# K1nght/Unified-Unlearning-w-Remain-Geometry

Hardware: AMD Instinct MI355X
Metric: SFR-on unlearning steps/sec, DiT-XL/2 256px bs32/GPU (higher is better)
Workload: dtype bf16

## Files before the change

include/sfron.h:

```cpp
#ifndef SFRON_H
#define SFRON_H
#include <stdint.h>
#ifdef __cplusplus
extern "C" {
#endif

int sfron_abi_version(void);
const char* sfron_build_arch(void);


int sfron_sweep_partials_len(void);

int sfron_sumsq_masked(const float* g, const float* g2, const uint8_t* mask, int64_t n, double* partials, int* nblk_out,
                       void* stream);

int sfron_sumsq_masked_ranges(const float* g, const uint8_t* mask, const int64_t* ranges, int n_ranges, double* partials, void* stream);

int sfron_clip_coef(const double* partials, int nblk, float max_norm, float* stats, void* stream);

int sfron_masked_clip_adam(float* p, const float* g, const float* g2 , float* m, float* v,
                           const uint8_t* mask, const float* stats,
                           int64_t n, double beta1, double beta2, double eps, double step_size, double bc2_sqrt,
                           double decay_mul, uint16_t* w_bf16, float* ema, double ema_decay, int ema_mode, void* stream);

// ... 39 lines not shown
int sfron_ddpm_alphas_cumprod(const float* betas, int T, float* abar, void* stream);
int sfron_ddpm_q_sample(const float* x0, const float* e, const int64_t* t, const float* abar, int n, int chw, float* x_t,
                        void* stream);
int sfron_ddpm_sample_loss(const float* e, const float* model_out, int n, int chw, float* per_sample, void* stream);
int sfron_ddpm_loss_coef(const float* per_sample, int n, int mode, float lambd, float scale, int n_global, float* wsum,
                         int use_wsum, float* coef, float* loss, void* stream);
int sfron_ddpm_loss_bwd(const float* e, const float* model_out, const float* coef, int n, int chw, float* d_model_out,
                        void* stream);
int sfron_ddim_step(const float* x, const float* eps, const float* noise, int64_t n, float s1, float s2, float s3, float c1,
                    float c2, float* x_next, float* x0_pred, void* stream);
int sfron_ddim_cfg_step(const float* x, const float* eps_uncond, const float* eps_cond, const float* noise, int64_t n, float guidance,
                        float sqrt_one_minus_at, float sqrt_at, float sqrt_a_prev, float dir_coef, float sigma, float* x_prev, float* pred_x0,
                        void* stream);

enum {
  SFRON_EPI_BF16 = 0,
  SFRON_EPI_F32 = 1,
  SFRON_EPI_GELU = 2,
  SFRON_EPI_GATE_RES = 3,
  SFRON_EPI_DGELU = 4,
  SFRON_EPI_POS = 5,
  SFRON_EPI_GELU_Q = 7,
  SFRON_EPI_DGELU_Q = 8,
  SFRON_EPI_QUICK_GELU = 9
};
typedef struct sfron_gemm_desc {
  const uint16_t* A; const uint16_t* B;
  int M, N, K, lda, ldb;
  int a_transposed, b_transposed;
  int epilogue;
  float alpha;
  const float* bias;
  uint16_t* c_bf16; int ldc_bf16;
  float* c_f32; int ldc_f32;
  uint16_t* aux; int ldaux;
  const float* gate; int ldgate;
  const float* pos;
  int tokens;
  int accumulate;
  const float* resid;
  int split_k;
  long split_stride;
  int tile_hint;
  float* a_rowsum;
  float* rowsum_ws;
  float* col_partials;
  const uint8_t* sumsq_mask;
  double* sumsq_partials;
} sfron_gemm_desc;
int sfron_gemm_bf16(const sfron_gemm_desc* desc , void* stream);
int sfron_gemm_dgelu_colpart_rows(int M, int N, int K);
int sfron_gemm_gelu_q_supported(int M, int N, int K);
int sfron_gemm_rowsum_supported(int M, int N, int K);
int sfron_split_sum_bf16(const float* slabs, int n_splits, int64_t n, int64_t split_stride, uint16_t* out, void* stream);
int sfron_split_gate_res(const float* slabs, int n_splits, int64_t split_stride, const float* bias, const float* gate, int ldgate, int tokens,
                         const float* resid, float* out, uint16_t* branch, int M, int N, void* stream);

int sfron_gemm_sumsq_partials(int M, int N, int K);



int sfron_fp8_quant_tensors(const float* params, const int64_t* table, int n_tensors, const float* scales, uint32_t* amax_bits,
                            uint8_t* dst, int mode, void* stream);
int sfron_fp8_update_scales(uint32_t* amax_bits, int n_tensors, float* scales, void* stream);
int sfron_fp8_activation_amax(uint32_t* act_amax, float* out3 , int reset, void* stream);

int sfron_cast_e4m3(const void* src, int src_is_bf16, int64_t n, float scale, uint8_t* dst, uint32_t* act_amax ,
                    void* stream);
int sfron_ln_modulate_fwd_q(const float* x, const float* shift, const float* scale, int ldmod, int tokens, int M, int D, uint16_t* out,
                            uint8_t* out_e4m3, float e4m3_scale, float* mean, float* rstd, uint32_t* act_amax ,
                            void* stream);

typedef struct sfron_fp8_gemm_desc {
  const uint8_t* A; const uint8_t* B;
  int M, N, K;
  const float* w_scale;
  float a_scale;
  int epilogue;
  const float* bias;
  uint16_t* c_bf16; int ldc_bf16;
  uint16_t* aux; int ldaux;
  uint8_t* c_e4m3; float c_e4m3_scale;
  float* c_f32; int ldc_f32;
  const float* resid;
  const float* gate; int ldgate;
  int tokens;
  uint32_t* act_amax;
  int aux_q;
} sfron_fp8_gemm_desc;
int sfron_fp8_gemm_supported(int M, int N, int K);
int sfron_fp8_gemm(const sfron_fp8_gemm_desc* desc , void* stream);

int sfron_cast_mx8(const uint16_t* src, int M, int N, uint8_t* dst, uint8_t* scales, void* stream);
int sfron_fp8_transpose_shadow(const uint8_t* w8, uint8_t* w8t, const int64_t* table, int n_matrices, void* stream);
typedef struct sfron_fp8_dgrad_desc {
  const uint8_t* A;
  const uint8_t* a_scales;
  const uint8_t* B;
  int M, N, K;
  const float* w_scale;
  int epilogue;
  uint16_t* c_bf16; int ldc_bf16;
  const uint16_t* aux; int ldaux;
  uint8_t* c_e4m3;
  uint8_t* c_scales;
  float* col_partials;
// ... 315 lines not shown
```

unified-unlearning-w-remain-geometry_amd/_lib.py:

```python
import ctypes
import os
from ctypes import POINTER, c_char_p, c_double, c_float, c_int, c_int64, c_void_p

_HERE = os.path.dirname(os.path.abspath(__file__))
LIB_PATH = os.path.join(_HERE, "libsfron.so")


class SfronError(RuntimeError):
    pass


_lib = None
ABI_VERSION = 16

_P = c_void_p
_S = c_void_p

_PROTOS = {
    "sfron_abi_version": (c_int, []),
    "sfron_build_arch": (c_char_p, []),
    "sfron_sweep_partials_len": (c_int, []),
    "sfron_sumsq_masked": (c_int, [_P, _P, _P, c_int64, _P, POINTER(c_int), _S]),
    "sfron_clip_coef": (c_int, [_P, c_int, c_float, _P, _S]),
    "sfron_masked_clip_adam": (c_int, [_P, _P, _P, _P, _P, _P, _P, c_int64, c_double, c_double, c_double, c_double, c_double,
                                       c_double, _P, _P, c_double, c_int, _S]),
    "sfron_masked_clip_adam_wg": (c_int, [_P, _P, _P, _P, _P, _P, _P, c_int64, c_double, c_double, c_double, c_double, c_double,
                                          c_double, _P, _P, c_double, c_int, c_int, _S]),
    "sfron_masked_clip_adam_q": (c_int, [_P, _P, _P, _P, _P, _P, c_int64, c_double, c_double, c_double, c_double, c_double, c_double, _P, _P,
                                         c_double, c_int, _P, _P, c_int, _S]),
    "sfron_sumsq_lowrank": (c_int, [_P, _P, c_int, c_int, c_int, _P, _P, POINTER(c_int), _S]),
    "sfron_adam_lowrank": (c_int, [_P, _P, _P, _P, _P, _P, _P, c_int, c_int, c_int, c_double, c_double, c_double, c_double, c_double,
                                   c_double, _P, _P, c_double, c_int, _S]),
    "sfron_ema_update": (c_int, [_P, _P, c_int64, c_double, c_int, _S]),
    "sfron_fisher_accum": (c_int, [_P, _P, c_int64, c_float, _S]),
    "sfron_fisher_accum_clipped": (c_int, [_P, _P, _P, _P, c_int64, c_float, _S]),
    "sfron_mask_from_fisher": (c_int, [_P, _P, c_int64, c_float, _P, _S]),
    "sfron_cast_bf16": (c_int, [_P, _P, c_int64, _S]),
    "sfron_q_sample": (c_int, [_P, _P, _P, _P, c_int, c_int, _P, _S]),
    "sfron_dit_loss_fwd_bwd": (c_int, [_P, _P, _P, _P, _P, c_int, c_int, c_int, c_float, _P, _P, _P, _S]),
    "sfron_p_sample": (c_int, [_P, _P, _P, _P, _P, c_int, c_int, c_int, c_int, _P, _P, _S]),
    "sfron_cfg_combine": (c_int, [_P, c_int, c_int, c_int, c_int, c_float, _S]),
    "sfron_ddim_step": (c_int, [_P, _P, _P, c_int64, c_float, c_float, c_float, c_float, c_float, _P, _P, _S]),
    "sfron_ddpm_alphas_cumprod": (c_int, [_P, c_int, _P, _S]),
    "sfron_ddpm_q_sample": (c_int, [_P, _P, _P, _P, c_int, c_int, _P, _S]),
    "sfron_ddpm_sample_loss": (c_int, [_P, _P, c_int, c_int, _P, _S]),
    "sfron_ddpm_loss_coef": (c_int, [_P, c_int, c_int, c_float, c_float, c_int, _P, c_int, _P, _P, _S]),
    "sfron_ddpm_loss_bwd": (c_int, [_P, _P, _P, c_int, c_int, _P, _S]),
}


class GemmDesc(ctypes.Structure):
    _fields_ = [("A", c_void_p), ("B", c_void_p),
                ("M", c_int), ("N", c_int), ("K", c_int), ("lda", c_int), ("ldb", c_int),
                ("a_transposed", c_int), ("b_transposed", c_int), ("epilogue", c_int), ("alpha", c_float),
                ("bias", c_void_p), ("c_bf16", c_void_p), ("ldc_bf16", c_int), ("c_f32", c_void_p), ("ldc_f32", c_int),
                ("aux", c_void_p), ("ldaux", c_int), ("gate", c_void_p), ("ldgate", c_int), ("pos", c_void_p),
                ("tokens", c_int), ("accumulate", c_int), ("resid", c_void_p), ("split_k", c_int),
                ("split_stride", ctypes.c_long), ("tile_hint", c_int), ("a_rowsum", c_void_p),
                ("rowsum_ws", c_void_p), ("col_partials", c_void_p), ("sumsq_mask", c_void_p), ("sumsq_partials", c_void_p)]


EPI_BF16, EPI_F32, EPI_GELU, EPI_GATE_RES, EPI_DGELU, EPI_POS = range(6)
EPI_GELU_Q, EPI_DGELU_Q = 7, 8
EPI_QUICK_GELU = 9

_PROTOS["sfron_gemm_bf16"] = (c_int, [POINTER(GemmDesc), _S])
_PROTOS["sfron_gemm_rowsum_supported"] = (c_int, [c_int, c_int, c_int])
_PROTOS["sfron_gemm_gelu_q_supported"] = (c_int, [c_int, c_int, c_int])
_PROTOS["sfron_gemm_sumsq_partials"] = (c_int, [c_int, c_int, c_int])
_PROTOS["sfron_split_sum_bf16"] = (c_int, [_P, c_int, c_int64, c_int64, _P, _S])
_PROTOS["sfron_split_gate_res"] = (c_int, [_P, c_int, c_int64, _P, _P, c_int, c_int, _P, _P, _P, c_int, c_int, _S])
_PROTOS["sfron_sumsq_masked_ranges"] = (c_int, [_P, _P, _P, c_int, _P, _S])
_PROTOS["sfron_gemm_dgelu_colpart_rows"] = (c_int, [c_int, c_int, c_int])
_PROTOS.update({
    "sfron_rows_per_chunk": (c_int, [c_int]),
    "sfron_ln_modulate_fwd": (c_int, [_P, _P, _P, c_int, c_int, c_int, c_int, _P, _P, _P, _S]),
    "sfron_ln_modulate_bwd": (c_int, [_P, _P, _P, _P, _P, c_int, c_int, c_int, c_int, _P, c_int, _P, _P, _S]),
    "sfron_gate_bwd": (c_int, [_P, _P, _P, c_int, c_int, c_int, c_int, _P, _P, _P, _S]),
    "sfron_ln_gate_bwd": (c_int, [_P, _P, _P, _P, _P, c_int, c_int, c_int, c_int, _P, c_int, _P, _P, _P, _P, c_int, _P, _P, _P, _S]),
    "sfron_reduce_chunks": (c_int, [_P, c_int, c_int, c_int, _P, c_int, c_int, _S]),
    "sfron_weighted_reduce": (c_int, [_P, c_int, c_int, c_int, _P, c_int, _P, _S]),
    "sfron_reduce_slots": (c_int, [_P, ctypes.c_long, c_int, c_int, c_int, c_int, POINTER(c_void_p), POINTER(ctypes.c_long),
                                   POINTER(c_int), _S]),
    "sfron_split_finish": (c_int, [_P, c_int64, c_int, c_int, _P, _P, c_int, _S]),
    "sfron_groupnorm_one_launch": (c_int, [c_int, c_int, c_int, c_int]),
    "sfron_groupnorm_fwd_src": (c_int, [_P, _P, _P, _P, c_int, c_int, c_int, c_int, c_float, c_int, _P, c_float, _P, _P, _P, _S]),
    "sfron_groupnorm_bwd_res_src": (c_int, [_P, _P, _P, c_int, _P, _P, _P, _P, c_int, c_int, c_int, c_int, c_int, _P, c_float, _P, c_int, c_int, _P,
                                            c_int, _P, _P, _S]),
    "sfron_groupnorm_bwd_cast_src": (c_int, [_P, _P, _P, c_int, _P, _P, _P, _P, c_int, c_int, c_int, c_int, c_int, _P, c_float, _P, _P, _P, _P, _S]),
    "sfron_reduce_batch": (c_int, [_P, c_int, _S]),
    "sfron_conv_wgrad_scatter_batch": (c_int, [_P, c_int, _S]),
    "sfron_reduce2": (c_int, [_P, _P, c_int, c_int, c_int, _P, c_int, _P, c_int, _S]),
    "sfron_gated_bias_grads": (c_int, [_P, _P, c_int, ctypes.c_long, ctypes.c_long, c_int, c_int, c_int, _P, ctypes.c_long,
                                       ctypes.c_long, ctypes.c_long, _S]),
    "sfron_colsum": (c_int, [_P, c_int, c_int, c_int, c_int, _P, c_int, _P, _S]),
    "sfron_timestep_embed": (c_int, [_P, c_int, c_int, _P, c_int, _S]),
    "sfron_latent_sample": (c_int, [_P, _P, c_int, c_int, c_int, c_float, _P, _S]),
    "sfron_vae_moments": (c_int, [_P, c_int, c_int, c_int, c_int, _P, _P, _P, _P, _P, c_float, _P, _S]),
    "sfron_vae_latent_in": (c_int, [_P, c_int, c_int, c_int, _P, _P, c_float, c_int, _P, _P, _S]),
    "sfron_guard_inputs": (c_int, [_P, _P, c_int, c_int, c_int, _P, _P, _P, _S]),
    "sfron_guard_finite": (c_int, [_P, _P, _P, _P, c_int, _P, _P, _S]),
    "sfron_silu_fwd": (c_int, [_P, c_int64, _P, _S]),
    "sfron_silu_bwd": (c_int, [_P, _P, c_int64, _P, _P, _S]),
    "sfron_cond_fwd": (c_int, [_P, _P, _P, _P, c_int, c_int, c_int, _P, _P, _S]),
    "sfron_cond_bwd": (c_int, [_P, _P, _P, _P, c_int, c_int, c_int, _P, _P, _S]),
    "sfron_patchify": (c_int, [_P, c_int, c_int, c_int, c_int, c_int, c_int, _P, c_int, _S]),
    "sfron_unpatchify": (c_int, [_P, c_int, c_int, c_int, c_int, c_int, c_int, _P, _S]),
    "sfron_attn_fwd": (c_int, [_P, _P, _P, c_int, c_int, c_int, c_int, _S]),
    "sfron_attn_bwd": (c_int, [_P, _P, _P, _P, _P, _P, c_int, c_int, c_int, c_int, _S]),
    "sfron_attn_bwd_form": (c_int, [c_int]),
    "sfron_attn_fwd_form": (c_int, [c_int]),
    "sfron_gemm_loader_waves": (c_int, [c_int]),
    "sfron_attn_bwd_bias_supported": (c_int, [c_int]),
    "sfron_attn_bwd_bias": (c_int, [_P, _P, _P, _P, _P, _P, c_int, c_int, c_int, c_int, _S]),
})


class Fp8GemmDesc(ctypes.Structure):
    _fields_ = [("A", c_void_p), ("B", c_void_p), ("M", c_int), ("N", c_int), ("K", c_int), ("w_scale", c_void_p), ("a_scale", c_float),
                ("epilogue", c_int), ("bias", c_void_p), ("c_bf16", c_void_p), ("ldc_bf16", c_int), ("aux", c_void_p), ("ldaux", c_int),
                ("c_e4m3", c_void_p), ("c_e4m3_scale", c_float), ("c_f32", c_void_p), ("ldc_f32", c_int), ("resid", c_void_p),
# ... 245 lines not shown
```

unified-unlearning-w-remain-geometry_amd/csrc/gemm.hip:

```cpp
#include "common.h"
#include "../../include/sfron.h"

extern int g_conv_loader_waves;
extern int g_fp8_loader_waves;
#include <atomic>

static inline bool need_attr(std::atomic<uint64_t>& mask) {
  int dev = 0;
  (void)hipGetDevice(&dev);
  const uint64_t bit = 1ull << (dev & 63);
  return (mask.fetch_or(bit) & bit) == 0;
}

struct GemmArgs {
  const __bf16* A; const __bf16* B;
  int M, N, K;
  int lda, ldb;
  __bf16* Cb; int ldcb;
  float* Cf; int ldcf;
  const float* bias;
  __bf16* aux; int ldaux;
  const float* gate; int ldgate;
  const float* pos;
  int T;
// ... 711 lines not shown
  }
  hipLaunchKernelGGL((k_gemm_fast<WM, WN, MT, NT, A_TR, B_TR, EPI, DBG>), dim3(g.ntm * g.ntn), dim3(WM * WN * 64), lds, s, g);
  hipError_t e = hipGetLastError();
  return e == hipSuccess ? SFRON_OK : (int)e;
}

}

__device__ __forceinline__ unsigned lds_addr(const __bf16* p) {
  return (unsigned)(uintptr_t)(__attribute__((address_space(3))) const char*)(const void*)p;
}
__device__ __forceinline__ bf16x4 asm_read_tr(unsigned addr) {
  bf16x4 r;
  asm volatile("ds_read_b64_tr_b16 %0, %1" : "=v"(r) : "v"(addr));
  return r;
}
__device__ __forceinline__ bf16x8 asm_read_b128(unsigned addr) {
  bf16x8 r;
  asm volatile("ds_read_b128 %0, %1" : "=v"(r) : "v"(addr));
  return r;
}
template <int OFF>
__device__ __forceinline__ bf16x4 asm_read_tr_off(unsigned addr) {
  bf16x4 r;
  asm volatile("ds_read_b64_tr_b16 %0, %1 offset:%2" : "=v"(r) : "v"(addr), "n"(OFF));
  return r;
}
template <int OFF>
__device__ __forceinline__ bf16x8 asm_read_b128_off(unsigned addr) {
  bf16x8 r;
  asm volatile("ds_read_b128 %0, %1 offset:%2" : "=v"(r) : "v"(addr), "n"(OFF));
  return r;
}
template <class F, int... I>
__device__ __forceinline__ void static_for_impl(F&& f, std::integer_sequence<int, I...>) { (f(std::integral_constant<int, I>{}), ...); }
template <int N, class F>
__device__ __forceinline__ void static_for(F&& f) { static_for_impl(f, std::make_integer_sequence<int, N>{}); }
#ifndef SFRON_RD_TAIL
#define SFRON_RD_TAIL 4
#endif
constexpr int op_span(int nops, int nm) {
  int span = nm - SFRON_RD_TAIL;
  const int min_span = (nops + 1) / 2;
  if (span < min_span) span = min_span;
  if (span > nm || SFRON_RD_TAIL <= 0) span = nm;
  return span < 1 ? 1 : span;
}
constexpr int op_cut(int i, int nops, int nm) { return i >= op_span(nops, nm) ? nops : i * nops / op_span(nops, nm); }
__device__ __forceinline__ void lds_reads_done() {
  asm volatile("s_waitcnt lgkmcnt(0)" ::: "memory");
  __builtin_amdgcn_sched_barrier(0);
}

template <int WM, int WN, int MT, int NT, bool A_TR, bool B_TR, int EPI, int SCHED = 0, int PRO = 2, bool BSUM = false, int NL = 0>
__global__ __launch_bounds__((WM * WN + NL) * 64) void k_gemm_pipe(GemmArgs g) {
  static_assert(!BSUM || (A_TR && B_TR && EPI == EPI_F32 && SCHED == 2), "row sums ride on the three-slot weight-gradient kernel");
  static_assert(NL == 0 || SCHED == 2, "loader waves feed the three-slot ring");
  static_assert(NL == 0 || !BSUM, "no row sums in the loader form");
  constexpr bool NL_SIMPLE = false;
  constexpr int FBM = WM * MT * 16, FBN = WN * NT * 16, NW = WM * WN;
  constexpr int FBM_P = A_TR ? tr_cols<FBM>() : FBM, FBN_P = B_TR ? tr_cols<FBN>() : FBN;
  constexpr int A_ELEMS = FBM_P * 64, B_ELEMS = FBN_P * 64;
  extern __shared__ __attribute__((aligned(16))) __bf16 smem[];
  constexpr int NS = SCHED == 2 ? 3 : 2;
  static_assert(NS == 2 || ((A_TR ? 2 * 2 * A_ELEMS + 64 * FBM_P < 65536 : 2 * A_ELEMS < 65536) && 2 * 2 * B_ELEMS + 64 * FBN_P < 65536),
                "ds offset field");
  auto sAp = [&](int b) { return smem + b * A_ELEMS; };
  auto sBp = [&](int b) { return smem + NS * A_ELEMS + b * B_ELEMS; };

  const int tid = threadIdx.x, lane = tid & 63;
  const int wave = __builtin_amdgcn_readfirstlane(tid >> 6);
#ifdef SFRON_DEBUG_KNOBS
  const long long clk_e = g.dbg_clk ? (long long)__builtin_amdgcn_s_memrealtime() : 0;
#endif
  const int wm = wave / WN, wn = wave % WN;
  const int nblk = gridDim.x;
  int id;
  {
    const int b = blockIdx.x, q = nblk >> 3, r = nblk & 7, x = b & 7, y = b >> 3;
    id = (x < r ? x * (q + 1) : r * (q + 1) + (x - r) * q) + y;
  }
  const int per_group = g.group_m * g.ntn;
  const int first_m = (id / per_group) * g.group_m;
  const int gsz = min(g.ntm - first_m, g.group_m);
  int tm = first_m + (id % per_group) % gsz, tn = (id % per_group) / gsz;
#ifdef SFRON_DEBUG_KNOBS
  if (g.dbg_same & 1) tm = 0;
  if (g.dbg_same & 2) tn = 0;
#endif
  const int m0 = tm * FBM, n0 = tn * FBN;

  f32x4 acc[MT][NT];
#pragma unroll
  for (int i = 0; i < MT; ++i)
#pragma unroll
    for (int j = 0; j < NT; ++j) acc[i][j] = f32x4{0.f, 0.f, 0.f, 0.f};
  if constexpr (SCHED >= 1) {
#pragma unroll
    for (int i = 0; i < MT; ++i)
#pragma unroll
      for (int j = 0; j < NT; ++j) { f32x4& c = acc[i][j]; asm volatile("" : "+v"(c)); }
  }
  f32x4 bacc[BSUM ? MT : 1];
  bf16x8 ones;
  const bool do_bs = BSUM && g.bsum != nullptr && wn == 0 && blockIdx.y == 0;
  int bs_c = g.ntn - 1;
  if constexpr (BSUM) {
#pragma unroll
// ... 466 lines not shown
        if (!wide) nt_store(reinterpret_cast<bf16x4*>(g.aux + (size_t)row * g.ldaux + col), ab[nt], g.nt_out & 1);
        const f32x4 x = as4(xr[mt & 1][nt]) + as4(gt[nt]) * v;
        if (pipe && mt + 1 < MT)
          xr[(mt + 1) & 1][nt] = *reinterpret_cast<const float4*>(g.resid + (size_t)(row + 16) * g.ldcf + col);
        *reinterpret_cast<f32x4*>(g.Cf + (size_t)row * g.ldcf + col) = x;
      }
#ifndef SFRON_TUNE_NO_BRANCH
      if (wide) {
        __bf16* const arow = g.aux + (size_t)row * g.ldaux;
#pragma unroll
        for (int np = 0; np < NP; ++np) *reinterpret_cast<uint4*>(arow + col_p + np * 32) = pair_pack(ab[2 * np], ab[2 * np + 1]);
        if constexpr (NT & 1) *reinterpret_cast<bf16x4*>(arow + col_b + (NT - 1) * 16) = ab[NT - 1];
      }
#endif
    }
  } else if constexpr (EPI == EPI_BF16 || EPI == EPI_GELU || EPI == EPI_GELUQ) {
    const bool wide = EPI == EPI_GELUQ || ((g.ldcb & 7) == 0 && (EPI != EPI_GELU || ((g.ldaux & 7) == 0 && !(g.nt_out & 1))));
    if (!wide) {
#pragma unroll
      for (int mt = 0; mt < MT; ++mt)
#pragma unroll
        for (int nt = 0; nt < NT; ++nt)
          epilogue_store<EPI>(g, row_b + mt * 16, col_b + nt * 16, acc[mt][nt],
                              PRE_BIAS ? &bias_v[PRE_BIAS ? nt : 0] : LATE_BIAS ? &bias_l[LATE_BIAS ? nt : 0] : nullptr);
    } else {
#pragma unroll
      for (int mt = 0; mt < MT; ++mt) {
        const int row = row_b + mt * 16;
        bf16x4 ob[NT], hb[EPI == EPI_GELU ? NT : 1];
        unsigned qb[EPI == EPI_GELUQ ? NT : 1];
#pragma unroll
        for (int nt = 0; nt < NT; ++nt) {
          f32x4 v = acc[mt][nt] * g.alpha;
          if constexpr (PRE_BIAS) v += as4(bias_v[nt]);
          else if constexpr (LATE_BIAS) v += as4(bias_l[nt]);
          else if (g.bias) v += as4(*reinterpret_cast<const float4*>(g.bias + col_b + nt * 16));
          if constexpr (EPI == EPI_GELU) {
            hb[nt] = f2bf4(v);
            ob[nt] = f2bf4(gelu_tanh4(v));
          } else if constexpr (EPI == EPI_GELUQ) {
            f32x4 y, dy;
            gelu_tanh_both4(v, y, dy);
            ob[nt] = f2bf4(y);
            qb[nt] = geluq_pack4(dy);
          } else {
            ob[nt] = f2bf4(v);
          }
        }
        __bf16* const crow = g.Cb + (size_t)row * g.ldcb;
#pragma unroll
        for (int np = 0; np < NP; ++np) *reinterpret_cast<uint4*>(crow + col_p + np * 32) = pair_pack(ob[2 * np], ob[2 * np + 1]);
        if constexpr (NT & 1) *reinterpret_cast<bf16x4*>(crow + col_b + (NT - 1) * 16) = ob[NT - 1];
        if constexpr (EPI == EPI_GELUQ) {
          static_assert(EPI != EPI_GELUQ || !(NT & 1), "byte-coded GELU': tile pairs only");
          uint8_t* const qrow = reinterpret_cast<uint8_t*>(g.aux) + (size_t)row * g.ldaux;
#pragma unroll
          for (int np = 0; np < NP; ++np) *reinterpret_cast<uint2*>(qrow + col_p + np * 32) = pair_pack8(qb[EPI == EPI_GELUQ ? 2 * np : 0], qb[EPI == EPI_GELUQ ? 2 * np + 1 : 0]);
        }
#ifndef SFRON_TUNE_NO_HPRE_STORE
        if constexpr (EPI == EPI_GELU) {
          __bf16* const arow = g.aux + (size_t)row * g.ldaux;
#pragma unroll
          for (int np = 0; np < NP; ++np) *reinterpret_cast<uint4*>(arow + col_p + np * 32) = pair_pack(hb[2 * np], hb[2 * np + 1]);
          if constexpr (NT & 1) *reinterpret_cast<bf16x4*>(arow + col_b + (NT - 1) * 16) = hb[NT - 1];
        }
#endif
      }
    }
  } else {
    [[maybe_unused]] float sq = 0.f;
    if constexpr (EPI == EPI_F32 && A_TR && B_TR && !BSUM) {
      if (g.sq_out) {
        uchar4 mk[MT][NT];
#pragma unroll
        for (int mt = 0; mt < MT; ++mt)
#pragma unroll
          for (int nt = 0; nt < NT; ++nt)
            mk[mt][nt] = g.sq_mask ? *reinterpret_cast<const uchar4*>(g.sq_mask + (size_t)(row_b + mt * 16) * g.ldcf + col_b + nt * 16)
                                   : make_uchar4(1, 1, 1, 1);
#pragma unroll
        for (int mt = 0; mt < MT; ++mt)
#pragma unroll
          for (int nt = 0; nt < NT; ++nt) {
            const f32x4 v = acc[mt][nt] * g.alpha;
            const uchar4 m4 = mk[mt][nt];
            sq += (m4.x ? v[0] * v[0] : 0.f) + (m4.y ? v[1] * v[1] : 0.f) + (m4.z ? v[2] * v[2] : 0.f) + (m4.w ? v[3] * v[3] : 0.f);
          }
      }
    }
#pragma unroll
    for (int mt = 0; mt < MT; ++mt)
#pragma unroll
      for (int nt = 0; nt < NT; ++nt)
        epilogue_store<EPI>(g, row_b + mt * 16, col_b + nt * 16, acc[mt][nt],
                            PRE_BIAS ? &bias_v[PRE_BIAS ? nt : 0] : LATE_BIAS ? &bias_l[LATE_BIAS ? nt : 0] : nullptr);
    if constexpr (EPI == EPI_F32 && A_TR && B_TR && !BSUM) {
      if (g.sq_out) {
        const double d = wave_sum_d((double)sq);
        __syncthreads();
        double* red = reinterpret_cast<double*>(smem);
        if (lane == 0) red[wave] = d;
        __syncthreads();
        if (tid == 0) {
          double t = red[0];
#pragma unroll
          for (int w2 = 1; w2 < NW; ++w2) t += red[w2];
          g.sq_out[blockIdx.x] = t;
        }
      }
    }
  }
#ifdef SFRON_DEBUG_KNOBS
  if (g.dbg_clk && tid == 0 && blockIdx.y == 0)
    g.dbg_clk[((A_TR ? 2 : B_TR ? 1 : 0) * 1024 + (blockIdx.x & 1023)) * 6 + 5] = (long long)__builtin_amdgcn_s_memrealtime();
#endif
}

#define SFRON_INST_PIPE(WM, WN, MT, NT)                                              \
  template __global__ void k_gemm_pipe<WM, WN, MT, NT, false, false, 0>(GemmArgs);  \
  template __global__ void k_gemm_pipe<WM, WN, MT, NT, false, false, 1>(GemmArgs);  \
  template __global__ void k_gemm_pipe<WM, WN, MT, NT, false, false, 2>(GemmArgs);  \
  template __global__ void k_gemm_pipe<WM, WN, MT, NT, false, false, 3>(GemmArgs);  \
  template __global__ void k_gemm_pipe<WM, WN, MT, NT, false, false, 5>(GemmArgs);  \
  template __global__ void k_gemm_pipe<WM, WN, MT, NT, false, true, 0>(GemmArgs);   \
  template __global__ void k_gemm_pipe<WM, WN, MT, NT, false, true, 1>(GemmArgs);   \
  template __global__ void k_gemm_pipe<WM, WN, MT, NT, false, true, 4>(GemmArgs);   \
  template __global__ void k_gemm_pipe<WM, WN, MT, NT, true, true, 0>(GemmArgs);    \
  template __global__ void k_gemm_pipe<WM, WN, MT, NT, true, true, 1>(GemmArgs);
SFRON_INST_PIPE(4, 2, 4, 6)
SFRON_INST_PIPE(4, 2, 3, 6)
SFRON_INST_PIPE(2, 2, 8, 6)
#undef SFRON_INST_PIPE
#define SFRON_INST_PIPE1(WM, WN, MT, NT)                                                \
  template __global__ void k_gemm_pipe<WM, WN, MT, NT, false, false, 0, 1>(GemmArgs);  \
  template __global__ void k_gemm_pipe<WM, WN, MT, NT, false, false, 1, 1>(GemmArgs);  \
  template __global__ void k_gemm_pipe<WM, WN, MT, NT, false, false, 2, 1>(GemmArgs);  \
  template __global__ void k_gemm_pipe<WM, WN, MT, NT, false, false, 3, 1>(GemmArgs);  \
  template __global__ void k_gemm_pipe<WM, WN, MT, NT, false, false, 5, 1>(GemmArgs);  \
  template __global__ void k_gemm_pipe<WM, WN, MT, NT, false, true, 0, 1>(GemmArgs);   \
  template __global__ void k_gemm_pipe<WM, WN, MT, NT, false, true, 1, 1>(GemmArgs);   \
  template __global__ void k_gemm_pipe<WM, WN, MT, NT, false, true, 4, 1>(GemmArgs);   \
  template __global__ void k_gemm_pipe<WM, WN, MT, NT, true, true, 0, 1>(GemmArgs);    \
  template __global__ void k_gemm_pipe<WM, WN, MT, NT, true, true, 1, 1>(GemmArgs);
SFRON_INST_PIPE1(4, 2, 4, 6)
SFRON_INST_PIPE1(4, 2, 3, 6)
#undef SFRON_INST_PIPE1
template __global__ void k_gemm_pipe<4, 2, 4, 6, false, false, EPI_GELUQ, 1>(GemmArgs);
template __global__ void k_gemm_pipe<4, 2, 4, 6, false, true, EPI_DGELUQ, 1>(GemmArgs);
template __global__ void k_gemm_pipe<4, 2, 3, 6, true, true, 0, 2>(GemmArgs);
template __global__ void k_gemm_pipe<4, 2, 3, 6, true, true, 1, 2>(GemmArgs);
template __global__ void k_gemm_pipe<4, 2, 3, 6, true, true, 1, 2, 2, true>(GemmArgs);
template __global__ void k_gemm_pipe<4, 2, 3, 6, false, false, 0, 2>(GemmArgs);
template __global__ void k_gemm_pipe<8, 1, 2, 9, false, false, 0, 2, 3>(GemmArgs);
template __global__ void k_gemm_pipe<8, 1, 2, 9, false, false, 1, 2, 3>(GemmArgs);
template __global__ void k_gemm_pipe<8, 1, 2, 9, false, false, 2, 2, 3>(GemmArgs);
template __global__ void k_gemm_pipe<8, 1, 2, 9, false, false, 3, 2, 3>(GemmArgs);
template __global__ void k_gemm_pipe<8, 1, 2, 9, false, false, 5, 2, 3>(GemmArgs);
template __global__ void k_gemm_pipe<8, 1, 2, 9, false, true, 0, 2, 3>(GemmArgs);
template __global__ void k_gemm_pipe<8, 1, 2, 9, false, true, 1, 2, 3>(GemmArgs);
template __global__ void k_gemm_pipe<8, 1, 2, 9, false, true, 4, 2, 3>(GemmArgs);
template __global__ void k_gemm_pipe<8, 1, 2, 9, false, false, 0, 2, 3, false, 4>(GemmArgs);
template __global__ void k_gemm_pipe<8, 1, 2, 9, false, false, 1, 2, 3, false, 4>(GemmArgs);
template __global__ void k_gemm_pipe<8, 1, 2, 9, false, false, 2, 2, 3, false, 4>(GemmArgs);
template __global__ void k_gemm_pipe<8, 1, 2, 9, false, false, 3, 2, 3, false, 4>(GemmArgs);
template __global__ void k_gemm_pipe<8, 1, 2, 9, false, false, 5, 2, 3, false, 4>(GemmArgs);
template __global__ void k_gemm_pipe<8, 1, 2, 9, false, true, 0, 2, 3, false, 4>(GemmArgs);
template __global__ void k_gemm_pipe<8, 1, 2, 9, false, true, 1, 2, 3, false, 4>(GemmArgs);
template __global__ void k_gemm_pipe<8, 1, 2, 9, false, true, 4, 2, 3, false, 4>(GemmArgs);
template __global__ void k_gemm_pipe<4, 2, 3, 6, true, true, 0, 2, 2, false, 4>(GemmArgs);
template __global__ void k_gemm_pipe<4, 2, 3, 6, false, false, 0, 2, 2, false, 4>(GemmArgs);
template __global__ void k_gemm_pipe<4, 2, 3, 6, true, true, 1, 2, 2, false, 4>(GemmArgs);

#ifdef SFRON_DEBUG_KNOBS
static long long* dbg_clk_buffer() {
  static long long* buf = [] {
    long long* p = nullptr;
    if (getenv("SFRON_GEMM_CLK") && hipMalloc(&p, 3 * 1024 * 6 * sizeof(long long)) == hipSuccess) (void)hipMemset(p, 0, 3 * 1024 * 6 * sizeof(long long));
    return p;
  }();
  return buf;
}
extern "C" int sfron_dbg_gemm_clock(double* mhz3, int* n3) {
  long long* d = dbg_clk_buffer();
  if (!d || !mhz3 || !n3) return SFRON_ERR_ARG;
  static long long host[3 * 1024 * 6];
  if (hipDeviceSynchronize() != hipSuccess || hipMemcpy(host, d, sizeof(host), hipMemcpyDeviceToHost) != hipSuccess) return (int)hipGetLastError();
  for (int c = 0; c < 3; ++c) {
    double v[1024]; int n = 0;
    for (int i = 0; i < 1024; ++i) { const long long dt = host[(c * 1024 + i) * 6], dr = host[(c * 1024 + i) * 6 + 1]; if (dr > 0) v[n++] = 100.0 * (double)dt / (double)dr; }
    for (int i = 1; i < n; ++i) { double x = v[i]; int j = i - 1; while (j >= 0 && v[j] > x) { v[j + 1] = v[j]; --j; } v[j + 1] = x; }
    mhz3[c] = n ? v[n / 2] : 0.0; n3[c] = n;
  }
  (void)hipMemset(d, 0, sizeof(host));
  return SFRON_OK;
}
extern "C" int sfron_dbg_gemm_phases(int cls, long long* out) {
  long long* d = dbg_clk_buffer();
  if (!d || !out || cls < 0 || cls > 2) return SFRON_ERR_ARG;
  if (hipDeviceSynchronize() != hipSuccess || hipMemcpy(out, d + (size_t)cls * 1024 * 6, 1024 * 6 * sizeof(long long), hipMemcpyDeviceToHost) != hipSuccess)
    return (int)hipGetLastError();
  (void)hipMemset(d + (size_t)cls * 1024 * 6, 0, 1024 * 6 * sizeof(long long));
  return SFRON_OK;
}
#endif

namespace {

template <int WM, int WN, int MT, int NT, bool A_TR, bool B_TR, int EPI, int SCHED = 0, int PRO = 2, bool BSUM = false, int NL = 0>
int launch_pipe(GemmArgs g, hipStream_t s) {
  constexpr int FBM = WM * MT * 16, FBN = WN * NT * 16;
  g.ntm = g.M / FBM; g.ntn = g.N / FBN;
#ifdef SFRON_DEBUG_KNOBS
  { static const int same = getenv("SFRON_GEMM_SAME_TILE") ? atoi(getenv("SFRON_GEMM_SAME_TILE")) : 0; g.dbg_same = same; }
  g.dbg_clk = dbg_clk_buffer();
#endif
  {
    const double per_xcd = (double)g.ntm * g.ntn / 8.0;
    int gm = 1;
    while (gm * 2 <= g.ntm && (double)(gm * 2) * (gm * 2) * FBM <= per_xcd * FBN * 1.5) gm *= 2;
    g.group_m = gm;
  }
  constexpr int NWD = NL > 0 ? NL : WM * WN;
  constexpr bool uneven = !GldsPlan<FBM, A_TR, NWD>::EVEN || !GldsPlan<FBN, B_TR, NWD>::EVEN;
  constexpr int FBM_P = A_TR ? tr_cols<FBM>() : FBM, FBN_P = B_TR ? tr_cols<FBN>() : FBN;
  const size_t lds = (SCHED == 2 ? 3 : 2) * (FBM_P + FBN_P) * 64 * sizeof(__bf16) + (uneven ? 1024 : 0);
  static std::atomic<uint64_t> done{0};
  if (need_attr(done)) {
    if (hipFuncSetAttribute(reinterpret_cast<const void*>(&k_gemm_pipe<WM, WN, MT, NT, A_TR, B_TR, EPI, SCHED, PRO, BSUM, NL>),
                            hipFuncAttributeMaxDynamicSharedMemorySize, (int)lds) != hipSuccess)
      return (int)hipGetLastError();
  }
  SFRON_LAUNCH_EV((k_gemm_pipe<WM, WN, MT, NT, A_TR, B_TR, EPI, SCHED, PRO, BSUM, NL>), dim3(g.ntm * g.ntn, cdiv(g.K, g.kchunk)), dim3((WM * WN + NL) * 64), lds, s, g);
  hipError_t e = hipGetLastError();
  return e == hipSuccess ? SFRON_OK : (int)e;
}

}

namespace {

constexpr int N_TILES = 9;
static const int TILE_BM[N_TILES] = {0, 128, 256, 256, 384, 192, 256, 192, 256};
static const int TILE_BN[N_TILES] = {0, 128, 192, 256, 192, 192, 192, 192, 144};
inline bool rowsum_ok(int M, int N, int K) {
  return M % 192 == 0 && N % 192 == 0 && K % 64 == 0 && K / 64 >= 2 && (K / 64 - 2) % 3 == 0;
}
inline bool tile_fits(const GemmArgs& g, int t) {
  return t >= 1 && t < N_TILES && g.M % TILE_BM[t] == 0 && g.N % TILE_BN[t] == 0;
}
inline int pick_fast_tile(const GemmArgs& g, int force, int transposed_operands) {
  if (g.K % 64 || force < 0) return 0;
  if (g.kchunk != g.K) {
    if (force == 32 || force == 35) return tile_fits(g, force - 30) ? force : 0;
    if (force != 0) return 0;
    if (transposed_operands == 2 && tile_fits(g, 5)) return 55;
    if (transposed_operands <= 1 && tile_fits(g, 2)) return 42;
    return 0;
  }
#ifdef SFRON_DEBUG_KNOBS
  if (force == 21 || force == 22) return tile_fits(g, 2) ? force : 0;
#endif
  if (force == 32 || force == 35 || force == 36) return tile_fits(g, force - 30) ? force : 0;
  if (force == 42 || force == 45) return tile_fits(g, force - 40) ? force : 0;
  if (force == 55) return tile_fits(g, 5) ? force : 0;
  if (force == 62) return tile_fits(g, 8) ? force : (tile_fits(g, 2) ? 42 : 0);
  if (force > 10) return 0;
  if (force > 0) return tile_fits(g, force) ? force : 0;
  auto eff = [&](int t) {
    const long tiles = (long)(g.M / TILE_BM[t]) * (g.N / TILE_BN[t]);
    return (double)tiles / (double)(((tiles + 255) / 256) * 256);
  };
  const bool even_nk = g.K % 128 == 0;
  if (transposed_operands == 2) return tile_fits(g, 5) ? 55 : 0;
#ifdef SFRON_DEBUG_KNOBS
  static const bool t62_all = getenv("SFRON_GEMM_T62_ALL") != nullptr;
#else
  constexpr bool t62_all = false;
#endif
  if (transposed_operands <= 1 && tile_fits(g, 8) && g.K % 192 == 0 && (t62_all || !tile_fits(g, 2) || eff(8) > eff(2) + 0.05)) return 62;
  if (tile_fits(g, 2) && eff(2) >= 0.5) return (transposed_operands == 1 || even_nk) ? 42 : 2;
  return (transposed_operands == 0 && tile_fits(g, 1)) ? 1 : 0;
}

int g_loader_waves = 4;

template <bool A_TR, bool B_TR, int EPI>
int launch_any(const GemmArgs& g, hipStream_t s, int force) {
  switch (pick_fast_tile(g, force, (A_TR ? 1 : 0) + (B_TR ? 1 : 0))) {
    case 1: return launch_fast<2, 2, 4, 4, A_TR, B_TR, EPI>(g, s);
    case 2: return launch_fast<4, 2, 4, 6, A_TR, B_TR, EPI>(g, s);
    case 3: return launch_fast<2, 4, 8, 4, A_TR, B_TR, EPI>(g, s);
    case 4: return launch_fast<4, 2, 6, 6, A_TR, B_TR, EPI>(g, s);
    case 5: return launch_fast<4, 2, 3, 6, A_TR, B_TR, EPI>(g, s);
    case 6: return launch_fast<2, 2, 8, 6, A_TR, B_TR, EPI>(g, s);
    case 7: return launch_fast<2, 2, 6, 6, A_TR, B_TR, EPI>(g, s);
    case 21: if constexpr (!A_TR && !B_TR && EPI == EPI_BF16) return launch_fast<4, 2, 4, 6, false, false, 0, 1>(g, s);
             else if constexpr (A_TR && B_TR && EPI == EPI_F32) return launch_fast<4, 2, 4, 6, true, true, 1, 1>(g, s); else return SFRON_ERR_UNSUPPORTED;
    case 22: if constexpr (!A_TR && !B_TR && EPI == EPI_BF16) return launch_fast<4, 2, 4, 6, false, false, 0, 2>(g, s);
             else if constexpr (A_TR && B_TR && EPI == EPI_F32) return launch_fast<4, 2, 4, 6, true, true, 1, 2>(g, s); else return SFRON_ERR_UNSUPPORTED;
    case 32: return launch_pipe<4, 2, 4, 6, A_TR, B_TR, EPI>(g, s);
    case 35: return launch_pipe<4, 2, 3, 6, A_TR, B_TR, EPI>(g, s);
    case 36: return launch_pipe<2, 2, 8, 6, A_TR, B_TR, EPI>(g, s);
    case 42: return (g.kchunk % 128 == 0 && g.K % g.kchunk == 0) ? launch_pipe<4, 2, 4, 6, A_TR, B_TR, EPI, 1>(g, s)
                                                                  : launch_pipe<4, 2, 4, 6, A_TR, B_TR, EPI>(g, s);
    case 45: return (g.kchunk % 128 == 0 && g.K % g.kchunk == 0) ? launch_pipe<4, 2, 3, 6, A_TR, B_TR, EPI, 1>(g, s)
                                                                  : launch_pipe<4, 2, 3, 6, A_TR, B_TR, EPI>(g, s);
    case 62:
      if constexpr ((!A_TR && !B_TR && (EPI == EPI_BF16 || EPI == EPI_F32 || EPI == EPI_GELU || EPI == EPI_GATE_RES || EPI == EPI_POS)) ||
                    (!A_TR && B_TR && (EPI == EPI_BF16 || EPI == EPI_F32 || EPI == EPI_DGELU))) {
        if (g.kchunk == g.K && g.K % 192 == 0)
          return (((g_loader_waves == 4 || g_loader_waves == 6) && B_TR) || g_loader_waves == 8) ? launch_pipe<8, 1, 2, 9, A_TR, B_TR, EPI, 2, 3, false, 4>(g, s) : launch_pipe<8, 1, 2, 9, A_TR, B_TR, EPI, 2, 3>(g, s);
      }
      if (!tile_fits(g, 2)) return launch<A_TR, B_TR, EPI>(g, s);
      return g.K % 128 == 0 && g.kchunk == g.K ? launch_pipe<4, 2, 4, 6, A_TR, B_TR, EPI, 1>(g, s) : launch_pipe<4, 2, 4, 6, A_TR, B_TR, EPI>(g, s);
    case 55:
      if constexpr (A_TR && B_TR && EPI == EPI_F32) {
        if (g.bsum) return rowsum_ok(g.M, g.N, g.K) && g.kchunk == g.K ? launch_pipe<4, 2, 3, 6, true, true, EPI_F32, 2, 2, true>(g, s) : SFRON_ERR_UNSUPPORTED;
      }
      if constexpr ((A_TR && B_TR && (EPI == EPI_BF16 || EPI == EPI_F32)) || (!A_TR && !B_TR && EPI == EPI_BF16)) {
        if (g.K % g.kchunk == 0 && (g.kchunk / 64) >= 2 && ((g.kchunk / 64) - 2) % 3 == 0) {
          if constexpr (A_TR && B_TR) { if (g_loader_waves == 4 || g_loader_waves == 5 || g_loader_waves == 8) return launch_pipe<4, 2, 3, 6, A_TR, B_TR, EPI, 2, 2, false, 4>(g, s); }
          if constexpr (!A_TR && !B_TR && EPI == EPI_BF16) { if (g_loader_waves == 7) return launch_pipe<4, 2, 3, 6, false, false, EPI_BF16, 2, 2, false, 4>(g, s); }
          return launch_pipe<4, 2, 3, 6, A_TR, B_TR, EPI, 2>(g, s);
        }
      }
      return (g.kchunk % 128 == 0 && g.K % g.kchunk == 0) ? launch_pipe<4, 2, 3, 6, A_TR, B_TR, EPI, 1>(g, s)
                                                           : launch_pipe<4, 2, 3, 6, A_TR, B_TR, EPI>(g, s);
    default: return launch<A_TR, B_TR, EPI>(g, s);
  }
}

template <int EPI>
int dispatch_layout(int a_tr, int b_tr, const GemmArgs& g, hipStream_t s, int force) {
  if (!a_tr && !b_tr) return launch_any<false, false, EPI>(g, s, force);
  if (!a_tr && b_tr) return launch_any<false, true, EPI>(g, s, force);
  if (a_tr && b_tr) return launch_any<true, true, EPI>(g, s, force);
  return SFRON_ERR_UNSUPPORTED;
}

}

extern "C" int sfron_gemm_rowsum_supported(int M, int N, int K) { return rowsum_ok(M, N, K) ? 1 : 0; }
extern "C" int sfron_gemm_gelu_q_supported(int M, int N, int K) { return M > 0 && N > 0 && K > 0 && M % 256 == 0 && N % 192 == 0 && K % 128 == 0 ? 1 : 0; }

extern "C" int sfron_gemm_sumsq_partials(int M, int N, int K) {
  if (M <= 0 || N <= 0 || K <= 0 || M % 192 || N % 192 || K % 64) return 0;
  return (M / 192) * (N / 192);
}

extern "C" int sfron_gemm_dgelu_colpart_rows(int M, int N, int K) {
  if (M <= 0 || N <= 0 || K <= 0) return 0;
  GemmArgs g{};
  g.M = M; g.N = N; g.K = K; g.kchunk = K;
  const int t = pick_fast_tile(g, 0, 1);
  if (t == 42) return M / 256;
  if (t == 62) return (K % 192 == 0 || tile_fits(g, 2)) ? M / 256 : 0;
  return 0;
}

int gemm_sumsq_lowrank(const uint16_t* a, const uint16_t* b, int R, int NM, int D, const uint8_t* mask, double* partials, int* nblk, void* stream) {
  GemmArgs g{};
  g.A = (const __bf16*)a; g.B = (const __bf16*)b;
  g.M = NM; g.N = D; g.K = R; g.lda = NM; g.ldb = D;
  g.alpha = 1.0f; g.kchunk = R; g.T = 1;
  g.ntm = cdiv(NM, BM); g.ntn = cdiv(D, BN);
  g.sq_mask = mask; g.sq_out = partials;
  *nblk = g.ntm * g.ntn;
  return launch<true, true, EPI_SUMSQ>(g, (hipStream_t)stream);
}

extern "C" int sfron_gemm_loader_waves(int n) {
  const int old = g_loader_waves;
#ifndef SFRON_DEBUG_KNOBS
  if (n != 0 && n != 4 && n != 9 && n != 10) return old;
#endif
  g_loader_waves = (n >= 9 && n <= 12) ? 4 : (n >= 4 && n <= 8) ? n : 0;
  g_fp8_loader_waves = n == 9 ? 4 : 0;
  g_conv_loader_waves = (n == 0 || n == 10) ? 0 : n == 11 ? 1 : n == 12 ? 2 : 3;
  return old;
}

extern "C"
int sfron_gemm_bf16(const sfron_gemm_desc* d, void* stream) {
  SFRON_CHECK_ARG(d && d->A && d->B && d->M > 0 && d->N > 0 && d->K > 0);
  SFRON_CHECK_ARG(d->N % 4 == 0 && d->lda % 8 == 0 && d->ldb % 8 == 0);
  if (!d->a_transposed || !d->b_transposed) SFRON_CHECK_ARG(d->K % 8 == 0);
  SFRON_CHECK_ARG((((uintptr_t)d->A | (uintptr_t)d->B) & 15) == 0);
  if (d->a_transposed) SFRON_CHECK_ARG(d->M % 8 == 0);
  if (d->b_transposed) SFRON_CHECK_ARG(d->N % 8 == 0);
  SFRON_CHECK_ARG(sfron_fits31(d->a_transposed ? sfron_extent(d->K, d->lda, d->M, 2) : sfron_extent(d->M, d->lda, d->K, 2)) &&
                  sfron_fits31(d->b_transposed ? sfron_extent(d->K, d->ldb, d->N, 2) : sfron_extent(d->N, d->ldb, d->K, 2)));
  GemmArgs g{};
  g.A = (const __bf16*)d->A; g.B = (const __bf16*)d->B;
  g.M = d->M; g.N = d->N; g.K = d->K; g.lda = d->lda; g.ldb = d->ldb;
  g.Cb = (__bf16*)d->c_bf16; g.ldcb = d->ldc_bf16;
  g.Cf = d->c_f32; g.ldcf = d->ldc_f32;
  g.bias = d->bias;
  g.aux = (__bf16*)d->aux; g.ldaux = d->ldaux;
  g.gate = d->gate; g.ldgate = d->ldgate;
  g.pos = d->pos; g.T = d->tokens > 0 ? d->tokens : 1;
  g.alpha = d->alpha; g.accumulate = d->accumulate;
  g.resid = d->resid ? d->resid : d->c_f32;
  g.kchunk = d->K; g.split_stride = 0;
  if (d->split_k > 1) {
    SFRON_CHECK_ARG(d->epilogue == SFRON_EPI_F32 && !d->bias && !d->accumulate && d->split_stride >= (long)d->M * d->ldc_f32);
    g.kchunk = cdiv(cdiv(d->K, d->split_k), BK) * BK;
    g.split_stride = d->split_stride;
  }
#ifdef SFRON_DEBUG_KNOBS
  static const int nt_mask = [] { const char* e = getenv("SFRON_GEMM_NT"); return e ? atoi(e) : 0; }();
#else
  constexpr int nt_mask = 0;
#endif
  g.nt_out = (nt_mask & 1) | ((nt_mask & 2) && d->a_transposed && d->b_transposed && d->split_k <= 1 && !d->accumulate ? 2 : 0);
  g.ntm = cdiv(d->M, BM); g.ntn = cdiv(d->N, BN);
  g.bsum = nullptr;
  g.colpart = nullptr;
  if (d->col_partials) {
    SFRON_CHECK_ARG((d->epilogue == SFRON_EPI_DGELU || d->epilogue == SFRON_EPI_DGELU_Q) && d->split_k <= 1 && d->tile_hint == 0);
    if (sfron_gemm_dgelu_colpart_rows(d->M, d->N, d->K) == 0) return SFRON_ERR_UNSUPPORTED;
    g.colpart = d->col_partials;
  }
  g.sq_mask = nullptr; g.sq_out = nullptr;
  if (d->sumsq_partials) {
    SFRON_CHECK_ARG(d->a_transposed && d->b_transposed && d->epilogue == SFRON_EPI_F32 && d->split_k <= 1 && d->tile_hint == 0 && !d->a_rowsum &&
                    !d->accumulate);
    if (sfron_gemm_sumsq_partials(d->M, d->N, d->K) == 0) return SFRON_ERR_UNSUPPORTED;
    g.sq_mask = d->sumsq_mask; g.sq_out = d->sumsq_partials;
  }
  if (d->a_rowsum) {
    SFRON_CHECK_ARG(d->rowsum_ws && d->a_transposed && d->b_transposed && d->epilogue == SFRON_EPI_F32 && d->split_k <= 1 &&
                    d->tile_hint == 0);
    if (!rowsum_ok(d->M, d->N, d->K)) return SFRON_ERR_UNSUPPORTED;
    g.bsum = d->rowsum_ws;
    const int rc = dispatch_layout<EPI_F32>(1, 1, g, (hipStream_t)stream, 0);
    if (rc != SFRON_OK) return rc;
    return sfron_reduce_chunks(d->rowsum_ws, 1, d->N / 192, d->M, d->a_rowsum, d->M, 0, stream);
  }
  hipStream_t s = (hipStream_t)stream;
  const int force = d->tile_hint;
  switch (d->epilogue) {
    case SFRON_EPI_BF16:
      SFRON_CHECK_ARG(g.Cb && g.ldcb % 4 == 0);
      return dispatch_layout<EPI_BF16>(d->a_transposed, d->b_transposed, g, s, force);
    case SFRON_EPI_F32:
      SFRON_CHECK_ARG(g.Cf && g.ldcf % 4 == 0);
      if (!d->a_transposed && !d->b_transposed && force == 0 && skinny_ok(g)) return launch_skinny(g, s);
      return dispatch_layout<EPI_F32>(d->a_transposed, d->b_transposed, g, s, force);
    case SFRON_EPI_GELU:
      SFRON_CHECK_ARG(g.Cb && g.aux && g.ldcb % 4 == 0 && g.ldaux % 4 == 0 && !d->a_transposed && !d->b_transposed);
      return launch_any<false, false, EPI_GELU>(g, s, force);
    case SFRON_EPI_GATE_RES:
      SFRON_CHECK_ARG(g.Cf && g.aux && g.gate && g.ldcf % 4 == 0 && g.ldaux % 4 == 0 && g.ldgate % 4 == 0 &&
                      !d->a_transposed && !d->b_transposed);
      return launch_any<false, false, EPI_GATE_RES>(g, s, force);
    case SFRON_EPI_DGELU:
      SFRON_CHECK_ARG(g.Cb && g.aux && g.ldcb % 4 == 0 && g.ldaux % 4 == 0 && !d->a_transposed && d->b_transposed);
      return launch_any<false, true, EPI_DGELU>(g, s, force);
    case SFRON_EPI_GELU_Q:
      SFRON_CHECK_ARG(g.Cb && g.aux && g.ldcb % 8 == 0 && g.ldaux % 8 == 0 && !d->a_transposed && !d->b_transposed && d->split_k <= 1 && force == 0);
      SFRON_CHECK_ARG((((uintptr_t)g.aux | (uintptr_t)g.Cb) & 15) == 0);
      if (!sfron_gemm_gelu_q_supported(d->M, d->N, d->K)) return SFRON_ERR_UNSUPPORTED;
      return launch_pipe<4, 2, 4, 6, false, false, EPI_GELUQ, 1>(g, s);
    case SFRON_EPI_DGELU_Q:
      SFRON_CHECK_ARG(g.Cb && g.aux && g.ldcb % 8 == 0 && g.ldaux % 8 == 0 && !d->a_transposed && d->b_transposed && d->split_k <= 1 && force == 0);
      SFRON_CHECK_ARG((((uintptr_t)g.aux | (uintptr_t)g.Cb) & 15) == 0);
      if (!sfron_gemm_gelu_q_supported(d->M, d->N, d->K)) return SFRON_ERR_UNSUPPORTED;
      return launch_pipe<4, 2, 4, 6, false, true, EPI_DGELUQ, 1>(g, s);
    case SFRON_EPI_QUICK_GELU:
      SFRON_CHECK_ARG(g.Cb && g.ldcb % 4 == 0 && !d->a_transposed && !d->b_transposed && d->split_k <= 1 && !d->accumulate);
      if ((force == 0 || force == 1) && d->K % 64 == 0 && tile_fits(g, 1)) return launch_fast<2, 2, 4, 4, false, false, EPI_QGELU>(g, s);
      return launch<false, false, EPI_QGELU>(g, s);
    case SFRON_EPI_POS:
      SFRON_CHECK_ARG(g.Cf && g.pos && g.ldcf % 4 == 0 && !d->a_transposed && !d->b_transposed);
      if (force == 0 && shortk_ok(g)) return launch_shortk(g, s);
      return launch_any<false, false, EPI_POS>(g, s, force);
    default:
      return SFRON_ERR_UNSUPPORTED;
  }
}
```

Measured before the change: 16.38.

## Add half-height 128x144 GEMM tile for two workgroups per CU

Adds a 4x1-wave pipelined GEMM variant with a 128x144 tile for forward-layout BF16 and quantized-GELU epilogues, sized so two workgroups fit in one CU's LDS. It is selectable by tile hint or by a compile-time tuning mask that defaults off. It also sets a waves-per-EU attribute on all pipelined GEMM kernels and handles odd tile counts in the byte-coded GELU store. The goal is better occupancy and latency hiding on large GEMMs, at the cost of less reuse per tile and possible register-pressure changes in existing kernels.

```diff
diff --git a/include/sfron.h b/include/sfron.h
--- a/include/sfron.h
+++ b/include/sfron.h
@@ -115,6 +115,8 @@
 int sfron_gemm_dgelu_colpart_rows(int M, int N, int K);
 int sfron_gemm_gelu_q_supported(int M, int N, int K);
 int sfron_gemm_rowsum_supported(int M, int N, int K);
+int sfron_gemm_half_tile(int M, int N, int K, int epilogue);
+int sfron_gemm_half_tile_lds_bytes(void);
 int sfron_split_sum_bf16(const float* slabs, int n_splits, int64_t n, int64_t split_stride, uint16_t* out, void* stream);
 int sfron_split_gate_res(const float* slabs, int n_splits, int64_t split_stride, const float* bias, const float* gate, int ldgate, int tokens,
                          const float* resid, float* out, uint16_t* branch, int M, int N, void* stream);
diff --git a/unified-unlearning-w-remain-geometry_amd/_lib.py b/unified-unlearning-w-remain-geometry_amd/_lib.py
--- a/unified-unlearning-w-remain-geometry_amd/_lib.py
+++ b/unified-unlearning-w-remain-geometry_amd/_lib.py
@@ -67,6 +67,8 @@
 _PROTOS["sfron_gemm_bf16"] = (c_int, [POINTER(GemmDesc), _S])
 _PROTOS["sfron_gemm_rowsum_supported"] = (c_int, [c_int, c_int, c_int])
 _PROTOS["sfron_gemm_gelu_q_supported"] = (c_int, [c_int, c_int, c_int])
+_PROTOS["sfron_gemm_half_tile"] = (c_int, [c_int, c_int, c_int, c_int])
+_PROTOS["sfron_gemm_half_tile_lds_bytes"] = (c_int, [])
 _PROTOS["sfron_gemm_sumsq_partials"] = (c_int, [c_int, c_int, c_int])
 _PROTOS["sfron_split_sum_bf16"] = (c_int, [_P, c_int, c_int64, c_int64, _P, _S])
 _PROTOS["sfron_split_gate_res"] = (c_int, [_P, c_int, c_int64, _P, _P, c_int, c_int, _P, _P, _P, c_int, c_int, _S])
diff --git a/unified-unlearning-w-remain-geometry_amd/csrc/gemm.hip b/unified-unlearning-w-remain-geometry_amd/csrc/gemm.hip
--- a/unified-unlearning-w-remain-geometry_amd/csrc/gemm.hip
+++ b/unified-unlearning-w-remain-geometry_amd/csrc/gemm.hip
@@ -787,8 +787,10 @@
   __builtin_amdgcn_sched_barrier(0);
 }
 
+constexpr int pipe_waves_per_simd(int wm, int wn, int nl) { return (wm == 4 && wn == 1) ? 2 : (wm * wn + nl + 3) / 4; }
 template <int WM, int WN, int MT, int NT, bool A_TR, bool B_TR, int EPI, int SCHED = 0, int PRO = 2, bool BSUM = false, int NL = 0>
-__global__ __launch_bounds__((WM * WN + NL) * 64) void k_gemm_pipe(GemmArgs g) {
+__global__ __launch_bounds__((WM * WN + NL) * 64) __attribute__((amdgpu_waves_per_eu(pipe_waves_per_simd(WM, WN, NL))))
+void k_gemm_pipe(GemmArgs g) {
   static_assert(!BSUM || (A_TR && B_TR && EPI == EPI_F32 && SCHED == 2), "row sums ride on the three-slot weight-gradient kernel");
   static_assert(NL == 0 || SCHED == 2, "loader waves feed the three-slot ring");
   static_assert(NL == 0 || !BSUM, "no row sums in the loader form");
@@ -1361,10 +1363,10 @@
         for (int np = 0; np < NP; ++np) *reinterpret_cast<uint4*>(crow + col_p + np * 32) = pair_pack(ob[2 * np], ob[2 * np + 1]);
         if constexpr (NT & 1) *reinterpret_cast<bf16x4*>(crow + col_b + (NT - 1) * 16) = ob[NT - 1];
         if constexpr (EPI == EPI_GELUQ) {
-          static_assert(EPI != EPI_GELUQ || !(NT & 1), "byte-coded GELU': tile pairs only");
           uint8_t* const qrow = reinterpret_cast<uint8_t*>(g.aux) + (size_t)row * g.ldaux;
 #pragma unroll
           for (int np = 0; np < NP; ++np) *reinterpret_cast<uint2*>(qrow + col_p + np * 32) = pair_pack8(qb[EPI == EPI_GELUQ ? 2 * np : 0], qb[EPI == EPI_GELUQ ? 2 * np + 1 : 0]);
+          if constexpr (NT & 1) *reinterpret_cast<unsigned*>(qrow + col_b + (NT - 1) * 16) = qb[EPI == EPI_GELUQ ? NT - 1 : 0];
         }
 #ifndef SFRON_TUNE_NO_HPRE_STORE
         if constexpr (EPI == EPI_GELU) {
@@ -1456,6 +1458,8 @@
 #undef SFRON_INST_PIPE1
 template __global__ void k_gemm_pipe<4, 2, 4, 6, false, false, EPI_GELUQ, 1>(GemmArgs);
 template __global__ void k_gemm_pipe<4, 2, 4, 6, false, true, EPI_DGELUQ, 1>(GemmArgs);
+template __global__ void k_gemm_pipe<4, 1, 2, 9, false, false, EPI_BF16, 1>(GemmArgs);
+template __global__ void k_gemm_pipe<4, 1, 2, 9, false, false, EPI_GELUQ, 1>(GemmArgs);
 template __global__ void k_gemm_pipe<4, 2, 3, 6, true, true, 0, 2>(GemmArgs);
 template __global__ void k_gemm_pipe<4, 2, 3, 6, true, true, 1, 2>(GemmArgs);
 template __global__ void k_gemm_pipe<4, 2, 3, 6, true, true, 1, 2, 2, true>(GemmArgs);
@@ -1532,7 +1536,8 @@
   constexpr int NWD = NL > 0 ? NL : WM * WN;
   constexpr bool uneven = !GldsPlan<FBM, A_TR, NWD>::EVEN || !GldsPlan<FBN, B_TR, NWD>::EVEN;
   constexpr int FBM_P = A_TR ? tr_cols<FBM>() : FBM, FBN_P = B_TR ? tr_cols<FBN>() : FBN;
-  const size_t lds = (SCHED == 2 ? 3 : 2) * (FBM_P + FBN_P) * 64 * sizeof(__bf16) + (uneven ? 1024 : 0);
+  constexpr size_t lds = (SCHED == 2 ? 3 : 2) * (FBM_P + FBN_P) * 64 * sizeof(__bf16) + (uneven ? 1024 : 0);
+  static_assert(!(WM == 4 && WN == 1) || 2 * lds <= 160 * 1024, "the half-height tile: two workgroups per CU");
   static std::atomic<uint64_t> done{0};
   if (need_attr(done)) {
     if (hipFuncSetAttribute(reinterpret_cast<const void*>(&k_gemm_pipe<WM, WN, MT, NT, A_TR, B_TR, EPI, SCHED, PRO, BSUM, NL>),
@@ -1556,6 +1561,24 @@
 }
 inline bool tile_fits(const GemmArgs& g, int t) {
   return t >= 1 && t < N_TILES && g.M % TILE_BM[t] == 0 && g.N % TILE_BN[t] == 0;
+}
+constexpr int HALF_BM = 128, HALF_BN = 144, HALF_MAX_K = 1152, HALF_SLOTS = 512, HALF_MIN_ROUNDS = 3;
+constexpr int HALF_LDS_BYTES = 2 * (HALF_BM + HALF_BN) * 64 * (int)sizeof(__bf16) + 1024;
+static_assert(2 * HALF_LDS_BYTES <= 160 * 1024 && HALF_LDS_BYTES <= 81920, "two half-height workgroups share a CU's LDS");
+inline bool half_tile_fits(int M, int N, int K) {
+  return M > 0 && N > 0 && K > 0 && M % HALF_BM == 0 && N % HALF_BN == 0 && K % 128 == 0 && K <= HALF_MAX_K;
+}
+#ifndef SFRON_TUNE_HALF_TILES
+#define SFRON_TUNE_HALF_TILES 0
+#endif
+inline bool half_tile_auto(int M, int N, int K, int epi) {
+  const int bit = epi == EPI_BF16 ? 1 : epi == EPI_GELUQ ? 2 : 0;
+  return (SFRON_TUNE_HALF_TILES & bit) && half_tile_fits(M, N, K) && (long)(M / HALF_BM) * (N / HALF_BN) >= (long)HALF_MIN_ROUNDS * HALF_SLOTS;
+}
+inline bool use_half_tile(const GemmArgs& g, int force, int epi) {
+  if (g.kchunk != g.K) return false;
+  if (force == 72) return half_tile_fits(g.M, g.N, g.K);
+  return force == 0 && half_tile_auto(g.M, g.N, g.K, epi);
 }
 inline int pick_fast_tile(const GemmArgs& g, int force, int transposed_operands) {
   if (g.K % 64 || force < 0) return 0;
@@ -1651,6 +1674,12 @@
 
 extern "C" int sfron_gemm_rowsum_supported(int M, int N, int K) { return rowsum_ok(M, N, K) ? 1 : 0; }
 extern "C" int sfron_gemm_gelu_q_supported(int M, int N, int K) { return M > 0 && N > 0 && K > 0 && M % 256 == 0 && N % 192 == 0 && K % 128 == 0 ? 1 : 0; }
+extern "C" int sfron_gemm_half_tile(int M, int N, int K, int epilogue) {
+  const int epi = epilogue == SFRON_EPI_BF16 ? EPI_BF16 : epilogue == SFRON_EPI_GELU_Q ? EPI_GELUQ : -1;
+  if (epi < 0 || !half_tile_fits(M, N, K)) return 0;
+  return half_tile_auto(M, N, K, epi) ? 2 : 1;
+}
+extern "C" int sfron_gemm_half_tile_lds_bytes(void) { return HALF_LDS_BYTES; }
 
 extern "C" int sfron_gemm_sumsq_partials(int M, int N, int K) {
   if (M <= 0 || N <= 0 || K <= 0 || M % 192 || N % 192 || K % 64) return 0;
@@ -1747,10 +1776,15 @@
     return sfron_reduce_chunks(d->rowsum_ws, 1, d->N / 192, d->M, d->a_rowsum, d->M, 0, stream);
   }
   hipStream_t s = (hipStream_t)stream;
-  const int force = d->tile_hint;
+  int force = d->tile_hint;
+  const bool fwd_layout = !d->a_transposed && !d->b_transposed;
   switch (d->epilogue) {
     case SFRON_EPI_BF16:
       SFRON_CHECK_ARG(g.Cb && g.ldcb % 4 == 0);
+      if (fwd_layout && (force == 0 || force == 71 || force == 72)) {
+        if (use_half_tile(g, force, EPI_BF16)) return launch_pipe<4, 1, 2, 9, false, false, EPI_BF16, 1>(g, s);
+        force = 0;
+      }
       return dispatch_layout<EPI_BF16>(d->a_transposed, d->b_transposed, g, s, force);
     case SFRON_EPI_F32:
       SFRON_CHECK_ARG(g.Cf && g.ldcf % 4 == 0);
@@ -1767,8 +1801,10 @@
       SFRON_CHECK_ARG(g.Cb && g.aux && g.ldcb % 4 == 0 && g.ldaux % 4 == 0 && !d->a_transposed && d->b_transposed);
       return launch_any<false, true, EPI_DGELU>(g, s, force);
     case SFRON_EPI_GELU_Q:
-      SFRON_CHECK_ARG(g.Cb && g.aux && g.ldcb % 8 == 0 && g.ldaux % 8 == 0 && !d->a_transposed && !d->b_transposed && d->split_k <= 1 && force == 0);
+      SFRON_CHECK_ARG(g.Cb && g.aux && g.ldcb % 8 == 0 && g.ldaux % 8 == 0 && !d->a_transposed && !d->b_transposed && d->split_k <= 1 &&
+                      (force == 0 || force == 71 || force == 72));
       SFRON_CHECK_ARG((((uintptr_t)g.aux | (uintptr_t)g.Cb) & 15) == 0);
+      if (use_half_tile(g, force, EPI_GELUQ)) return launch_pipe<4, 1, 2, 9, false, false, EPI_GELUQ, 1>(g, s);
       if (!sfron_gemm_gelu_q_supported(d->M, d->N, d->K)) return SFRON_ERR_UNSUPPORTED;
       return launch_pipe<4, 2, 4, 6, false, false, EPI_GELUQ, 1>(g, s);
     case SFRON_EPI_DGELU_Q:
```

After: 16.16. 1.3% lower.
